# dvnam1605/MAACO-path-planing

Hardware: NVIDIA B200
Metric: path evals/sec (MAACO ant tours, MPA/PSO/GA fitness) at 1/2/4/8 B200 vs CPU (higher is better)
Workload: dtype f64

## Files before the change

maaco_path_planing_b200/csrc/mpp_maaco.cu:

```cuda
#include <type_traits>
#include <cmath>
#include <cstdlib>
#include <thread>
#include <vector>

#include "mpp_common.cuh"

static inline double hdist(int r0, int c0, int r1, int c1) {
    long long dr = r0 - r1, dc = c0 - c1;
    return std::sqrt((double)(dr * dr + dc * dc));
}

extern "C" double mpp_maaco_q0(int K, int k, double q0_initial) {
    double k0 = 0.7 * (double)K, q0;
    if ((double)k < k0) {
        if (std::fabs((double)K - k0) < 1e-6) q0 = q0_initial;
        else q0 = ((double)(K - k) / (double)K) * q0_initial;
    } else {
        double q0_at_k0 = (((double)K - k0) / (double)K) * q0_initial;
        q0 = q0_at_k0 +
             (((double)k - k0) / ((double)K - k0 + 1e-9)) * (q0_initial * (1 - ((double)K - k0) / (double)K) / 2.0);
    }
    q0 = q0 > 0.01 ? q0 : 0.01;
    return q0 < 0.99 ? q0 : 0.99;
}

static void host_tables(int R, int C, int start, int target, const mpp_maaco_params *p, double *tau0, double *E01,
                        double *dt) {
    const int sr = start / C, sc = start % C, tr = target / C, tc = target % C;
    double dsT = hdist(sr, sc, tr, tc);
    if (dsT < 1e-9) dsT = 1e-9;
    auto work = [&](int r_lo, int r_hi) {
        for (int r = r_lo; r < r_hi; ++r)
            for (int c = 0; c < C; ++c) {
                const size_t i = (size_t)r * C + c;
                const double diT = hdist(r, c, tr, tc);
                const double dsi = hdist(sr, sc, r, c);
                dt[i] = diT;
                {
                    const double den = dsi + diT;
                    double factor;
                    if (den < 1e-9) factor = (dsi < 1e-6 || diT < 1e-6) ? 1.0 : 0.1;
                    else factor = dsT / den;
                    const double v = factor * p->C0_initial_pheromone;
                    tau0[i] = v < 1e-9 ? 1e-9 : v;
                }
                double h;
                if (dsT < 1e-9) h = p->wh_min;
                else h = p->wh_max - (p->wh_max - p->wh_min) * std::exp(-p->k_h_adaptive * diT / dsT);
                const double g = 1.0 - h;
                const double base = g * dsi + h * diT;
                double d0 = base + p->a_turn_coef * 0.0, d1 = base + p->a_turn_coef * 1.0;
                d0 = d0 > 1e-9 ? d0 : 1e-9;
                d1 = d1 > 1e-9 ? d1 : 1e-9;
                E01[2 * i] = std::pow(1.0 / d0, p->beta);
                E01[2 * i + 1] = std::pow(1.0 / d1, p->beta);
            }
    };
    unsigned nt = std::thread::hardware_concurrency();
    if (nt > 16) nt = 16;
    if (nt < 2 || (size_t)R * C < 65536) {
        work(0, R);
    } else {
        std::vector<std::thread> th;
        int per = (R + (int)nt - 1) / (int)nt;
        for (unsigned t = 0; t < nt; ++t) {
            int lo = (int)t * per, hi = lo + per > R ? R : lo + per;
            if (lo < hi) th.emplace_back(work, lo, hi);
        }
        for (auto &t : th) t.join();
    }
}

__global__ void mpp_maaco_tau0_kernel(const double *__restrict__ tau0_free, const uint32_t *__restrict__ occ, int occ_words,
                                      int pitch, int R, int C, double *__restrict__ tau, long long tau_stride) {
    const int i = blockIdx.x * blockDim.x + threadIdx.x;
    if (i >= R * C) return;
    occ += (size_t)blockIdx.y * occ_words;
    const int r = i / C, pb = i % C + 1;
    const bool obst = (occ[(r + 1) * pitch + (pb >> 5)] >> (pb & 31)) & 1u;
    tau[(size_t)blockIdx.y * tau_stride + i] = obst ? 1e-9 : tau0_free[i];
}

extern "C" int mpp_maaco_tables(const mpp_map_batch *maps, const mpp_maaco_params *p, double *tau0_dev, long long tau_stride,
                                double *E01_dev, double *dist_t_dev, void *stream) {
    MPP_REQUIRE(maps && p && tau0_dev && E01_dev, "mpp_maaco_tables: null argument");
    const int R = maps->rows, C = maps->cols;
    const size_t n = (size_t)R * C;
    MPP_REQUIRE(tau_stride >= (long long)n, "mpp_maaco_tables: tau_stride < rows*cols");
    const MppMapMeta &M0 = maps->meta_host[0];
    MPP_REQUIRE(M0.start >= 0 && M0.target >= 0, "mpp_maaco_tables: map has no start/target");
    for (int k = 1; k < maps->n_maps; ++k)
        MPP_REQUIRE(maps->meta_host[k].start == M0.start && maps->meta_host[k].target == M0.target,
                    "mpp_maaco_tables: the maps of a batch must share start and target (map %d differs); group them", k);
    std::vector<double> buf(4 * n);
    double *tau0 = buf.data(), *E01 = tau0 + n, *dt = E01 + 2 * n;
    host_tables(R, C, M0.start, M0.target, p, tau0, E01, dt);
    cudaStream_t s = (cudaStream_t)stream;
    MPP_CUDA(cudaSetDevice(maps->device));
    double *tau0_free = nullptr;
    MPP_CUDA(cudaMalloc(&tau0_free, n * 8));
    MPP_CUDA(cudaMemcpyAsync(tau0_free, tau0, n * 8, cudaMemcpyHostToDevice, s));
    MPP_CUDA(cudaMemcpyAsync(E01_dev, E01, 2 * n * 8, cudaMemcpyHostToDevice, s));
    if (dist_t_dev) MPP_CUDA(cudaMemcpyAsync(dist_t_dev, dt, n * 8, cudaMemcpyHostToDevice, s));
    mpp_maaco_tau0_kernel<<<dim3(((int)n + 255) / 256, maps->n_maps), 256, 0, s>>>(
        tau0_free, maps->occ_dev, maps->occ_words, maps->pitch_words, R, C, tau0_dev, tau_stride);
    MPP_CUDA(cudaGetLastError());
    MPP_CUDA(cudaStreamSynchronize(s));
    MPP_CUDA(cudaFree(tau0_free));
    return MPP_OK;
}

struct RankLayout { size_t margin, fast_words, bundle_words, nb8_words, total_words; };
static RankLayout rank_layout(int R, int C) {
    RankLayout L;
    L.margin = (size_t)(C + 2) * 9;
    L.fast_words = ((size_t)9 * R * C + 2 * L.margin + 1) & ~(size_t)1;
    L.bundle_words = (L.fast_words + (size_t)18 * R * C + 3) & ~(size_t)3;
    L.nb8_words = L.bundle_words + (size_t)4 * R * C;
    L.total_words = L.nb8_words + (size_t)2 * R * C;
    return L;
}
static inline int tiles_r(int R) { return (R + 31) >> 5; }
static inline int tiles_c(int C) { return (C + 31) >> 5; }

extern "C" long long mpp_maaco_rank_words(int rows, int cols) { return (long long)rank_layout(rows, cols).total_words; }
extern "C" long long mpp_maaco_slab_words(int tile_rows, int cols, int n_ants) {
    return (long long)tile_rows * tiles_c(cols) * (long long)n_ants * 32;
}
extern "C" long long mpp_maaco_touched_words(int tile_rows, int cols, int n_ants) {
    return 2ll * tile_rows * tiles_c(cols) * ((n_ants + 31) / 32);
}

#define MPP_MAX_PEERS 16
struct TourArgs {
    const MppMapMeta *meta;
    const uint32_t *rank;
    size_t rank_stride, rank_margin, rank_fast_words, rank_bundle_words, rank_nb8_words;
    int R, C;
    const double *tau, *E01;
    size_t tau_stride, E01_stride;
    uint32_t it;
    double q0, alpha;
    int n_ants, ant_offset;
    const uint64_t *seeds;
    uint32_t *slabs, *touched;
    size_t slab_stride, touched_stride;
    uint8_t *moves;
    int max_cells;
    mpp_ant_result *result;
    size_t result_stride;
    unsigned long long *steps;
    const int32_t *latch;
};
struct TourPeers {
    uint32_t *peer_slabs[MPP_MAX_PEERS];
    uint32_t *peer_touched[MPP_MAX_PEERS];
    mpp_ant_result *peer_result[MPP_MAX_PEERS];
    int n_peers, rows_per_rank;
    int n_total;
};

#define MPP_SQRT2 1.4142135623730951
#ifndef MPP_TOUR1_THREADS
#define MPP_TOUR1_THREADS 128
#endif

__device__ __noinline__ double pow_slow(double x, double y) { return pow(x, y); }

__device__ __noinline__ int tour_select_slow(uint32_t cand, int cr, int cc, int C, bool have_prev, int prev_m,
                                             const double *__restrict__ tau, const double *__restrict__ E01,
                                             double alpha, double q0, double u0, double u1) {
    int mv[8], n = 0;
    double attr[8];
#pragma unroll
    for (int m = 0; m < 8; ++m) {
        if (!((cand >> m) & 1u)) continue;
        const int dr = (int)((0xA940u >> (2 * m)) & 3u) - 1, dc = (int)((0x9224u >> (2 * m)) & 3u) - 1;
        const int j = (cr + dr) * C + (cc + dc);
        const bool turn = have_prev && (m != prev_m);
        const double tv = tau[j];
        const double ta = (alpha == 1.0) ? tv : pow_slow(tv, alpha);
        attr[n] = ta * E01[2 * (size_t)j + (turn ? 1 : 0)];
        mv[n] = m;
        ++n;
    }
    int k;
    if (u0 <= q0) {
        double mx = -1.0;
        int best[8], nb = 0;
        for (int i = 0; i < n; ++i) {
            if (attr[i] > mx) { mx = attr[i]; nb = 0; best[nb++] = i; }
            else if (fabs(attr[i] - mx) < 1e-9) best[nb++] = i;
        }
        int q = (int)(u1 * (double)nb);
        q = q < nb ? q : nb - 1;
        k = best[q];
    } else {
        double S = 0.0;
        for (int i = 0; i < n; ++i) S += attr[i];
        bool uniform = S < 1e-9;
        double pr[8];
        double ps = 0.0;
        if (!uniform) {
            for (int i = 0; i < n; ++i) { pr[i] = attr[i] / S; ps += pr[i]; }
            if (fabs(ps - 1.0) > 1e-6) {
                const double ps0 = ps;
                ps = 0.0;
                for (int i = 0; i < n; ++i) { pr[i] = pr[i] / ps0; ps += pr[i]; }
            }
            if (!(fabs(ps - 1.0) <= 1.4901161193847656e-08)) uniform = true;
        }
        if (uniform) {
            k = (int)(u1 * (double)n);
        } else {
            double cdf[8], acc = 0.0;
            for (int i = 0; i < n; ++i) { acc += pr[i]; cdf[i] = acc; }
            k = 0;
            for (int i = 0; i < n; ++i)
                if (cdf[i] / acc <= u1) ++k;
        }
        k = k < n ? k : n - 1;
    }
    return mv[k];
}

struct TourSlabs {
    uint32_t *slabs, *touched;
    size_t n_ants;
    int NW, TR, TC;
    const TourPeers *peers;
    int rows_per_rank, ant_offset, NW_total;
    size_t n_total, peer_touched_off;
};
__device__ __forceinline__ uint32_t tour_tile_load(const TourSlabs &V, int a, int trow, int tcx, int lane) {
    if (trow < 0 || trow >= V.TR || tcx < 0 || tcx >= V.TC) return 0u;
    const int tile = trow * V.TC + tcx;
    uint32_t tw = 0u;
    if (lane == 0) tw = __ldcg(V.touched + (size_t)tile * V.NW + (a >> 5));
    tw = __shfl_sync(0xffffffffu, tw, 0);
    if (!((tw >> (a & 31)) & 1u)) return 0u;
    return __ldcg(V.slabs + ((size_t)tile * V.n_ants + a) * 32 + lane);
}
__device__ __forceinline__ void tour_tile_store(const TourSlabs &V, int a, int trow, int tcx, int lane, uint32_t v) {
    if (trow < 0 || trow >= V.TR || tcx < 0 || tcx >= V.TC) return;
    if (!__any_sync(0xffffffffu, v != 0u)) return;
    const int tile = trow * V.TC + tcx;
    V.slabs[((size_t)tile * V.n_ants + a) * 32 + lane] = v;
    if (lane == 0) atomicOr(V.touched + (size_t)tile * V.NW + (a >> 5), 1u << (a & 31));
    if (V.peers) {
        const int g = trow / V.rows_per_rank, tl = (trow - g * V.rows_per_rank) * V.TC + tcx;
        const size_t ga = (size_t)V.ant_offset + a;
        V.peers->peer_slabs[g][((size_t)tl * V.n_total + ga) * 32 + lane] = v;
        if (lane == 0) atomicOr(V.peers->peer_touched[g] + V.peer_touched_off + (size_t)tl * V.NW_total + (ga >> 5), 1u << (ga & 31));
    }
}

__device__ __forceinline__ uint32_t ldg32_pinned(const uint32_t *p) {
    uint32_t v;
    asm volatile("ld.volatile.global.u32 %0, [%1];" : "=r"(v) : "l"(p) : "memory");
    return v;
}
__device__ __forceinline__ uint2 lds_u2(uint32_t addr) {
    uint2 v;
    asm volatile("ld.shared.v2.u32 {%0, %1}, [%2];" : "=r"(v.x), "=r"(v.y) : "r"(addr));
    return v;
}
__device__ __forceinline__ uint32_t lds_u8(uint32_t addr) {
    uint32_t v;
    asm volatile("ld.shared.u8 %0, [%1];" : "=r"(v) : "r"(addr));
    return v;
}
__device__ __forceinline__ uint32_t lds_u32(uint32_t addr) {
// ... 366 lines not shown
                            pool = cand & ~((1u << best) - 1u);
                        }
                        const int n = __popc(pool);
                        const int k = (pack >> (3 * n - 3)) & 7u;
                        m = (int)lds_u8(sbase_k + T1_KTH_OFF + pool * 8u + (uint32_t)k);
                    }
                    const uint4 mvv = lds_u4(sbase_k + T1_MOVE_OFF + 16u * (uint32_t)m);
                    dcur = (int)mvv.x; dpr = (int)mvv.y; dcc = (int)mvv.z; dphi = (int)mvv.w;
                    dl = lds_f64(sbase_k + T1_DLEN_OFF + 8u * (uint32_t)m);
                    if (fast_ok) {
                        const uint32_t by = (((m & 4) ? nb.y : nb.x) >> (8 * (m & 3))) & 0xFFu;
                        const uint32_t fl = lds_u32(sbase_k + T1_FLD_OFF + 4u * (by >> 4));
                        const uint32_t A3n = (by >> 1) & 7u;
                        const uint32_t Gn = A3n ? ((fl >> (3u * (A3n - 1u))) & 7u) : 0u;
                        fw2 = (by & 1u) | (A3n << 1) | (fl << 4) | (Gn << 25);
                    }
                }
            }
            if (active) {
                cur += dcur;
                if (fast_ok) bq = ldg128_pinned(bundle + cur);
                gap -= dphi;
                gap = gap > 0 ? gap : 0;
                prow_s += (uint32_t)dpr;
                lrow += dpr >> 3;
                lcol += dcc;
                asm volatile("red.shared.or.b32 [%0], %1;" ::"r"(prow_s + 4u * ((uint32_t)lcol >> 5)), "r"(1u << (lcol & 31)) : "memory");
                if (n_path <= k_max_cells) *mvp = (uint8_t)m;
                ++mvp;
                len += dl;
                if (m != prev_m) ++turns;
                prev_m = m;
                ++n_path;
                if (cur == k_target || n_path >= k_max_path) active = false;
#ifdef MPP_TOUR_STATS
                st_c1 = clock64();
#endif
            }
        }
    }
    for (int src = 0; src < apw && a0 + src < A.n_ants; ++src) {
        const int s_wr = __shfl_sync(0xffffffffu, wr, src), s_wc = __shfl_sync(0xffffffffu, wc, src);
        const uint2 o0 = win_w[src * 64 + lane], o1 = win_w[src * 64 + lane + 32];
        tour_tile_store(V, a0 + src, s_wr, s_wc, lane, o0.x);
        tour_tile_store(V, a0 + src, s_wr, s_wc + 1, lane, o0.y);
        tour_tile_store(V, a0 + src, s_wr + 1, s_wc, lane, o1.x);
        tour_tile_store(V, a0 + src, s_wr + 1, s_wc + 1, lane, o1.y);
    }
    if (lane < apw && a < A.n_ants) {
        const bool ok = !failed && cur == target;
        mpp_ant_result res;
        res.length = ok ? len : __longlong_as_double(0x7ff0000000000000ll);
        res.n_cells = ok ? n_path : 0;
        res.turns = ok ? (turns > 0 ? turns : 0) : -1;
        A.result[(size_t)map * A.result_stride + A.ant_offset + a] = res;
        if constexpr (P2P)
            for (int g = 0; g < PA.n_peers; ++g) PA.peer_result[g][A.ant_offset + a] = res;
        if (A.steps) atomicAdd(A.steps, (unsigned long long)(n_path - 1));
#ifdef MPP_TOUR_STATS
        int *st = (int *)(A.moves + ((size_t)map * A.n_ants + a + 1) * A.max_cells - 32);
        st[0] = st_t1; st[1] = st_t2; st[2] = st_t3; st[3] = st_slides; st[4] = (int)(st_c1 - st_c0); st[5] = n_path - 1;
        st[6] = ok ? 1 : 0;
#endif
    }
}

static int colony_check(const mpp_map_batch *maps, const mpp_colony *c, const char *who) {
    MPP_REQUIRE(maps && c, "%s: null argument", who);
    MPP_REQUIRE(c->tau && c->E01 && c->rank && c->slabs && c->touched && c->moves && c->result && c->deposit && c->okbits &&
                    c->state && c->best_cells && c->seeds, "%s: null colony buffer", who);
    MPP_REQUIRE(c->max_cells > 0 && c->tau_stride >= (long long)maps->rows * maps->cols, "%s: bad max_cells / tau_stride", who);
    for (int k = 0; k < maps->n_maps; ++k)
        MPP_REQUIRE(maps->meta_host[k].start >= 0 && maps->meta_host[k].target >= 0, "%s: map %d has no start/target", who, k);
    return MPP_OK;
}

static int tours_launch(const mpp_map_batch *maps, const mpp_colony *c, int iteration, double q0, double alpha,
                        int n_ants, int ant_offset, int n_ants_total, int ants_per_warp,
                        uint32_t *const *peer_slabs, uint32_t *const *peer_touched, mpp_ant_result *const *peer_result,
                        int n_peers, int rows_per_rank, void *stream) {
    int rc = colony_check(maps, c, "mpp_maaco_tours");
    if (rc) return rc;
    MPP_REQUIRE(n_ants > 0 && ant_offset >= 0 && ant_offset + n_ants <= n_ants_total, "mpp_maaco_tours: bad ant range");
    MPP_CUDA(cudaSetDevice(maps->device));
    const RankLayout L = rank_layout(maps->rows, maps->cols);
    const int TR = tiles_r(maps->rows);
    TourArgs A;
    A.meta = maps->meta_dev;
    A.rank = c->rank; A.rank_stride = L.total_words; A.rank_margin = L.margin; A.rank_fast_words = L.fast_words;
    A.rank_bundle_words = L.bundle_words; A.rank_nb8_words = L.nb8_words;
    A.R = maps->rows; A.C = maps->cols;
    A.tau = c->tau; A.tau_stride = (size_t)c->tau_stride; A.E01 = c->E01; A.E01_stride = (size_t)c->E01_stride;
    A.it = (uint32_t)iteration; A.q0 = q0; A.alpha = alpha;
    A.n_ants = n_ants; A.ant_offset = ant_offset;
    A.seeds = c->seeds;
    const size_t tw = (size_t)mpp_maaco_touched_words(TR, maps->cols, n_ants) / 2;
    A.slabs = c->slabs; A.slab_stride = (size_t)mpp_maaco_slab_words(TR, maps->cols, n_ants);
    A.touched = c->touched + (size_t)(iteration & 1) * tw * maps->n_maps; A.touched_stride = tw;
    A.moves = c->moves; A.max_cells = c->max_cells;
    A.result = c->result; A.result_stride = (size_t)n_ants_total;
    A.steps = c->steps; A.latch = c->latch;
    TourPeers PA;
    for (int g = 0; g < MPP_MAX_PEERS; ++g) {
        PA.peer_slabs[g] = g < n_peers ? peer_slabs[g] : nullptr;
        PA.peer_touched[g] = g < n_peers ? peer_touched[g] : nullptr;
        PA.peer_result[g] = g < n_peers ? peer_result[g] : nullptr;
    }
    PA.n_peers = n_peers; PA.rows_per_rank = rows_per_rank; PA.n_total = n_ants_total;
    int apw = 16;
    const char *e = getenv("MPP_TOUR_APW");
    if (e) apw = atoi(e);
    else if (ants_per_warp) apw = ants_per_warp;
    else {
        const long long total = (long long)n_ants * maps->n_maps;
        while (apw > 2 && (total + apw - 1) / apw < 12ll * maps->sm_count) apw >>= 1;
    }
    MPP_REQUIRE(apw == 1 || apw == 2 || apw == 4 || apw == 8 || apw == 16 || apw == 32,
                "ants per warp (MPP_TOUR_APW / ants_per_warp) must be a power of two <= 32");
    const int warps = (n_ants + apw - 1) / apw, wpb = MPP_TOUR1_THREADS / 32;
    const size_t smem = T1_WIN_OFF + (size_t)wpb * apw * 512;
    {
        static size_t smem_set[64] = {0};
        const int dv = maps->device & 63;
        if (smem > smem_set[dv]) {
            MPP_CUDA(cudaFuncSetAttribute(mpp_maaco_tour1_kernel<false>, cudaFuncAttributeMaxDynamicSharedMemorySize, (int)smem));
            MPP_CUDA(cudaFuncSetAttribute(mpp_maaco_tour1_kernel<true>, cudaFuncAttributeMaxDynamicSharedMemorySize, (int)smem));
            smem_set[dv] = smem;
        }
    }
    const dim3 grid((warps + wpb - 1) / wpb, maps->n_maps);
    if (n_peers > 0) mpp_maaco_tour1_kernel<true><<<grid, MPP_TOUR1_THREADS, smem, (cudaStream_t)stream>>>(A, apw, PA);
    else mpp_maaco_tour1_kernel<false><<<grid, MPP_TOUR1_THREADS, smem, (cudaStream_t)stream>>>(A, apw, TourNoPeers());
    MPP_CUDA(cudaGetLastError());
    return MPP_OK;
}

extern "C" int mpp_maaco_tours(const mpp_map_batch *maps, const mpp_colony *c, int iteration, double q0, double alpha,
                               int n_ants, int ant_offset, int n_ants_total, int ants_per_warp, void *stream) {
    return tours_launch(maps, c, iteration, q0, alpha, n_ants, ant_offset, n_ants_total, ants_per_warp, nullptr, nullptr,
                        nullptr, 0, 1, stream);
}

extern "C" int mpp_maaco_tours_p2p(const mpp_map_batch *maps, const mpp_colony *c, int iteration, double q0, double alpha,
                                   int n_ants, int ant_offset, int n_ants_total, int ants_per_warp,
                                   uint32_t *const *slabs_peers, uint32_t *const *touched_peers,
                                   mpp_ant_result *const *result_peers, int n_peers, int tile_rows_per_rank, void *stream) {
    MPP_REQUIRE(maps && maps->n_maps == 1, "mpp_maaco_tours_p2p: a sharded colony is one map");
    MPP_REQUIRE(slabs_peers && touched_peers && result_peers && n_peers > 0 && n_peers <= MPP_MAX_PEERS && tile_rows_per_rank > 0 &&
                    (long long)n_peers * tile_rows_per_rank >= tiles_r(maps->rows), "mpp_maaco_tours_p2p: bad peer arguments");
    return tours_launch(maps, c, iteration, q0, alpha, n_ants, ant_offset, n_ants_total, ants_per_warp, slabs_peers,
                        touched_peers, result_peers, n_peers, tile_rows_per_rank, stream);
}

__global__ void __launch_bounds__(128) mpp_maaco_rank_kernel(const uint8_t *__restrict__ svalid_all,
                                                             const double *__restrict__ tau_all, size_t tau_stride,
                                                             const double *__restrict__ E01_all, size_t E01_stride,
                                                             double alpha, int R, int C,
                                                             const MppMapMeta *__restrict__ meta, uint32_t *__restrict__ rank_all,
                                                             size_t rank_stride, size_t rank_margin, size_t rank_fast_words,
                                                             size_t rank_bundle_words, size_t rank_nb8_words,
                                                             const int32_t *__restrict__ latch) {
    const int cell = blockIdx.x * 128 + threadIdx.x;
    if (cell >= R * C) return;
    if (latch && *latch) return;
    const int map = blockIdx.y;
    const uint8_t *svalid = svalid_all + (size_t)map * R * C;
    const double *tau = tau_all + (size_t)map * tau_stride;
    const double *E01 = E01_all + (size_t)map * E01_stride;
    uint32_t *rank_fast = rank_all + (size_t)map * rank_stride + rank_margin;
    uint2 *rank_slow = (uint2 *)(rank_all + (size_t)map * rank_stride + rank_fast_words);
    uint32_t *bundle = rank_all + (size_t)map * rank_stride + rank_bundle_words;
    uint8_t *nb8 = (uint8_t *)(rank_all + (size_t)map * rank_stride + rank_nb8_words);
    const uint32_t P1 = meta[map].s1.P1;
    const uint32_t sv = svalid[cell];
    double a0[8], a1[8];
#pragma unroll
    for (int m = 0; m < 8; ++m) {
        a0[m] = a1[m] = -1.0;
        if ((sv >> m) & 1u) {
            const int j = cell + ((int)((0xA940u >> (2 * m)) & 3u) - 1) * C + ((int)((0x9224u >> (2 * m)) & 3u) - 1);
            const double tv = tau[j];
            const double ta = (alpha == 1.0) ? tv : pow_slow(tv, alpha);
            const double2 e = *(const double2 *)(E01 + 2 * (size_t)j);
            a0[m] = ta * e.x;
            a1[m] = ta * e.y;
        }
    }
    const bool p1_three = __popc(P1) == 3;
    const int s0 = __ffs(P1) - 1, s1 = __ffs(P1 & (P1 - 1)) - 1, s2 = 31 - __clz(P1);
    for (int ctx = 0; ctx < 9; ++ctx) {
        double a[8];
#pragma unroll
        for (int m = 0; m < 8; ++m) a[m] = (ctx > 0 && m != ctx - 1) ? a1[m] : a0[m];
        double cmx = 0.0;
#pragma unroll
        for (int m = 0; m < 8; ++m) cmx = fmax(cmx, a[m]);
        uint32_t word = 0xFFFFFFu, perm = 0u, fast = 7u, order = 0u;
        if (cmx < 1e-10) {
            word = 0u;
#pragma unroll
            for (int m = 0; m < 8; ++m) {
                int pos = 0;
#pragma unroll
                for (int q = 0; q < 8; ++q) pos += (a[q] > a[m]) || (a[q] == a[m] && q < m);
                word |= (uint32_t)pos << (3 * m);
                perm |= (uint32_t)m << (4 * pos);
            }
            fast = 0u;
            if (p1_three) {
                const uint32_t p0 = (word >> (3 * s0)) & 7u, p1 = (word >> (3 * s1)) & 7u, p2 = (word >> (3 * s2)) & 7u;
                order = (p0 < p1 ? 1u : 0u) | (p0 < p2 ? 2u : 0u) | (p1 < p2 ? 4u : 0u);
#pragma unroll
                for (uint32_t c = 1; c < 8; ++c) {
                    uint32_t bp = 8u, bi = 0u;
                    if ((c & 1u) && p0 < bp) { bp = p0; bi = 0u; }
                    if ((c & 2u) && p1 < bp) { bp = p1; bi = 1u; }
                    if ((c & 4u) && p2 < bp) { bp = p2; bi = 2u; }
                    fast |= (c & ~((1u << bi) - 1u)) << (3u * c);
                }
            }
        }
        const size_t t = (size_t)cell * 9 + ctx;
        rank_fast[t] = fast | (sv << 24);
        rank_slow[t] = make_uint2(perm, word | (sv << 24));
        if (p1_three && ctx > 0) {
            const int mv = ctx - 1;
            const int pr = cell / C - ((int)((0xA940u >> (2 * mv)) & 3u) - 1), pc = cell % C - ((int)((0x9224u >> (2 * mv)) & 3u) - 1);
            if (pr >= 0 && pr < R && pc >= 0 && pc < C) {
                const uint32_t A3 = ((sv >> s0) & 1u) | (((sv >> s1) & 1u) << 1) | (((sv >> s2) & 1u) << 2);
                nb8[((size_t)pr * C + pc) * 8 + mv] = (uint8_t)((fast & 7u ? 1u : 0u) | (A3 << 1) | (order << 4));
                const int k = (ctx == s0 + 1) ? 0 : ((ctx == s1 + 1) ? 1 : ((ctx == s2 + 1) ? 2 : -1));
                if (k >= 0) bundle[((size_t)pr * C + pc) * 4 + k] = tour_word2(fast | (sv << 24), s0, s1, s2);
            }
        }
    }
}

extern "C" int mpp_maaco_rank(const mpp_map_batch *maps, const mpp_colony *c, double alpha, void *stream) {
    int rc = colony_check(maps, c, "mpp_maaco_rank");
    if (rc) return rc;
    MPP_CUDA(cudaSetDevice(maps->device));
    const int total = maps->rows * maps->cols;
    const RankLayout L = rank_layout(maps->rows, maps->cols);
    mpp_maaco_rank_kernel<<<dim3((total + 127) / 128, maps->n_maps), 128, 0, (cudaStream_t)stream>>>(
        maps->svalid_dev, c->tau, (size_t)c->tau_stride, c->E01, (size_t)c->E01_stride, alpha, maps->rows, maps->cols,
        maps->meta_dev, c->rank, L.total_words, L.margin, L.fast_words, L.bundle_words, L.nb8_words, c->latch);
    MPP_CUDA(cudaGetLastError());
    return MPP_OK;
}

#define MPP_BEST_THREADS 1024
__device__ __forceinline__ bool lt_len_idx(double la, int ia, double lb, int ib) {
    return la < lb || (la == lb && ia < ib);
}
__device__ __forceinline__ int move_delta(uint32_t m, int C) {
    return ((int)((0xA940u >> (2 * m)) & 3u) - 1) * C + ((int)((0x9224u >> (2 * m)) & 3u) - 1);
}

__global__ void __launch_bounds__(MPP_BEST_THREADS)
mpp_maaco_best_kernel(const mpp_ant_result *__restrict__ res_all, const uint8_t *__restrict__ moves_all, int max_cells,
                      int moves_ant_offset, int moves_n_ants, int n, double Q, int iteration, int C,
                      const MppMapMeta *__restrict__ meta, mpp_maaco_state *state_all, int32_t *best_cells_all,
                      double *deposit_all, uint32_t *okbits_all, double *log_all, int log_rows,
                      const int32_t *__restrict__ latch) {
    __shared__ double s_len[32];
    __shared__ int s_idx[32];
    __shared__ int s_t[32];
    __shared__ double b_len;
    __shared__ int b_r, b_ant, b_turns, b_copy, s_base;
    if (latch && *latch) return;
    const int map = blockIdx.x;
    const mpp_ant_result *res = res_all + (size_t)map * n;
    double *deposit = deposit_all + (size_t)map * n;
    uint32_t *okbits = okbits_all + (size_t)map * ((n + 31) >> 5);
    mpp_maaco_state *state = state_all + map;
    const int tid = threadIdx.x, lane = tid & 31, wid = tid >> 5;
    const double INF = __longlong_as_double(0x7ff0000000000000ll);
    double ml = INF;
    int mi = 0x7fffffff;
    for (int i0 = 0; i0 < n; i0 += MPP_BEST_THREADS) {
        const int i = i0 + tid;
        bool dep = false;
        if (i < n) {
            const mpp_ant_result ri = res[i];
            const double l = ri.length;
            if (lt_len_idx(l, i, ml, mi)) { ml = l; mi = i; }
            dep = (l != INF && ri.n_cells > 0 && l > 1e-6);
            deposit[i] = dep ? Q / l : 0.0;
        }
        const uint32_t ok = __ballot_sync(0xffffffffu, dep);
        if (lane == 0 && i < n) okbits[i >> 5] = ok;
    }
#pragma unroll
    for (int o = 16; o; o >>= 1) {
        const double ol = __shfl_xor_sync(0xffffffffu, ml, o);
        const int oi = __shfl_xor_sync(0xffffffffu, mi, o);
        if (lt_len_idx(ol, oi, ml, mi)) { ml = ol; mi = oi; }
    }
    if (lane == 0) { s_len[wid] = ml; s_idx[wid] = mi; }
    __syncthreads();
    if (wid == 0) {
        ml = s_len[lane]; mi = s_idx[lane];
#pragma unroll
        for (int o = 16; o; o >>= 1) {
            const double ol = __shfl_xor_sync(0xffffffffu, ml, o);
            const int oi = __shfl_xor_sync(0xffffffffu, mi, o);
            if (lt_len_idx(ol, oi, ml, mi)) { ml = ol; mi = oi; }
        }
        if (lane == 0) { b_len = ml; b_r = mi; }
    }
    __syncthreads();
    const double L = b_len;
    const int r = b_r;
    int bt = 0x7fffffff, bi = 0x7fffffff;
    if (L != INF) {
        for (int i = tid; i < n; i += MPP_BEST_THREADS) {
            if (i < r) continue;
            const mpp_ant_result ri = res[i];
            const double l = ri.length;
            if (i == r || fabs(l - L) < 1e-9) {
                const int t = ri.turns;
                if (t >= 0 && (t < bt || (t == bt && i < bi))) { bt = t; bi = i; }
            }
        }
    }
#pragma unroll
    for (int o = 16; o; o >>= 1) {
        const int ot = __shfl_xor_sync(0xffffffffu, bt, o), oi = __shfl_xor_sync(0xffffffffu, bi, o);
        if (ot < bt || (ot == bt && oi < bi)) { bt = ot; bi = oi; }
    }
    if (lane == 0) { s_t[wid] = bt; s_idx[wid] = bi; }
    __syncthreads();
    if (wid == 0) {
        bt = s_t[lane]; bi = s_idx[lane];
#pragma unroll
        for (int o = 16; o; o >>= 1) {
            const int ot = __shfl_xor_sync(0xffffffffu, bt, o), oi = __shfl_xor_sync(0xffffffffu, bi, o);
            if (ot < bt || (ot == bt && oi < bi)) { bt = ot; bi = oi; }
        }
        if (lane == 0) {
            const bool any = (L != INF);
            b_ant = any ? bi : -1;
            b_turns = any ? bt : -1;
            mpp_maaco_state st = *state;
            int copy = 0;
            if (any) {
                if (L < st.best_len) {
                    st.best_len = L; st.best_turns = bt; copy = 1;
                } else if (fabs(L - st.best_len) < 1e-9) {
                    if (bt < st.best_turns) { st.best_turns = bt; copy = 1; }
                }
            }
            if (copy) { st.best_n_cells = res[bi].n_cells; st.best_iter = iteration; st.best_ant = bi; }
            st.iter_best_len = L; st.iter_best_turns = b_turns; st.iter_best_ant = b_ant;
            *state = st;
            b_copy = copy;
            if (log_all && iteration >= 1 && iteration <= log_rows) {
                double *lg = log_all + ((size_t)map * log_rows + (size_t)(iteration - 1)) * 4;
                lg[0] = L; lg[1] = (double)b_turns; lg[2] = st.best_len; lg[3] = (double)st.best_turns;
            }
        }
    }
    __syncthreads();
    if (b_copy && b_ant >= moves_ant_offset && b_ant < moves_ant_offset + moves_n_ants) {
        const int a = b_ant - moves_ant_offset;
        int nm = res[b_ant].n_cells - 1;
        if (nm > max_cells) nm = max_cells;
        const uint8_t *mv = moves_all + ((size_t)map * moves_n_ants + a) * max_cells;
        int32_t *out = best_cells_all + (size_t)map * (max_cells + 1);
        if (tid == 0) { out[0] = meta[map].start; s_base = meta[map].start; }
        __syncthreads();
        for (int k0 = 0; k0 < nm; k0 += MPP_BEST_THREADS) {
            const int k = k0 + tid;
            int x = (k < nm) ? move_delta(mv[k], C) : 0;
#pragma unroll
            for (int o = 1; o < 32; o <<= 1) { const int y = __shfl_up_sync(0xffffffffu, x, o); if (lane >= o) x += y; }
            if (lane == 31) s_idx[wid] = x;
            __syncthreads();
            if (wid == 0) {
                int w = s_idx[lane];
#pragma unroll
                for (int o = 1; o < 32; o <<= 1) { const int y = __shfl_up_sync(0xffffffffu, w, o); if (lane >= o) w += y; }
                s_idx[lane] = w;
            }
            __syncthreads();
            const int cell = s_base + (wid ? s_idx[wid - 1] : 0) + x;
            if (k < nm) out[k + 1] = cell;
            __syncthreads();
            if (tid == MPP_BEST_THREADS - 1) s_base = cell;
            __syncthreads();
        }
    }
}

extern "C" int mpp_maaco_best(const mpp_map_batch *maps, const mpp_colony *c, int moves_ant_offset, int moves_n_ants,
                              int n_ants_total, double Q, int iteration, void *stream) {
    int rc = colony_check(maps, c, "mpp_maaco_best");
// ... 481 lines not shown
```

Baseline: 5.982 million.

## Tile MAACO rank kernel in shared memory with incremental ranking and coalesced stores

Rewrites the rank kernel to process 32x8 cell tiles. Each block stages tau^alpha*E01 products in shared memory with a halo, so each neighbour's product is computed once per tile rather than once per adjacent cell. The per-context 8x8 rank comparison is replaced by precomputed rank words with an incremental fix-up for the changed move. Outputs are staged in shared memory so fast/slow rank words and nb8/bundle entries go out as coalesced row writes instead of scattered byte stores. This costs a halo recompute for border cells, extra shared memory and more register pressure, and the logic is intricate enough to risk ranking mismatches.

```diff
diff --git a/maaco_path_planing_b200/csrc/mpp_maaco.cu b/maaco_path_planing_b200/csrc/mpp_maaco.cu
--- a/maaco_path_planing_b200/csrc/mpp_maaco.cu
+++ b/maaco_path_planing_b200/csrc/mpp_maaco.cu
@@ -118,7 +118,7 @@
     L.fast_words = ((size_t)9 * R * C + 2 * L.margin + 1) & ~(size_t)1;
     L.bundle_words = (L.fast_words + (size_t)18 * R * C + 3) & ~(size_t)3;
     L.nb8_words = L.bundle_words + (size_t)4 * R * C;
-    L.total_words = L.nb8_words + (size_t)2 * R * C;
+    L.total_words = (L.nb8_words + (size_t)2 * R * C + 3) & ~(size_t)3;
     return L;
 }
 static inline int tiles_r(int R) { return (R + 31) >> 5; }
@@ -791,7 +791,26 @@
                         touched_peers, result_peers, n_peers, tile_rows_per_rank, stream);
 }
 
-__global__ void __launch_bounds__(128) mpp_maaco_rank_kernel(const uint8_t *__restrict__ svalid_all,
+#define RANK_TW 32
+#define RANK_TH 8
+#define RANK_EW (RANK_TW + 2)
+#define RANK_EH (RANK_TH + 2)
+#define RANK_AW (RANK_TW + 4)
+#define RANK_AH (RANK_TH + 4)
+#ifndef MPP_RANK_MINB
+#define MPP_RANK_MINB 4
+#endif
+
+__device__ __forceinline__ int rank_beats(double aq, double am, bool q_lower) { return q_lower ? (aq >= am) : (aq > am); }
+
+__device__ __forceinline__ uint32_t rank_word2_of_byte(uint32_t by, const uint32_t *fields) {
+    const uint32_t A3 = (by >> 1) & 7u;
+    if (by & 1u) return 1u | (A3 << 1);
+    const uint32_t f = fields[by >> 4];
+    return (A3 << 1) | (f << 4) | ((A3 ? (f >> (3u * (A3 - 1u))) & 7u : 0u) << 25);
+}
+
+__global__ void __launch_bounds__(RANK_TW * RANK_TH, MPP_RANK_MINB) mpp_maaco_rank_kernel(const uint8_t *__restrict__ svalid_all,
                                                              const double *__restrict__ tau_all, size_t tau_stride,
                                                              const double *__restrict__ E01_all, size_t E01_stride,
                                                              double alpha, int R, int C,
@@ -799,89 +818,188 @@
                                                              size_t rank_stride, size_t rank_margin, size_t rank_fast_words,
                                                              size_t rank_bundle_words, size_t rank_nb8_words,
                                                              const int32_t *__restrict__ latch) {
-    const int cell = blockIdx.x * 128 + threadIdx.x;
-    if (cell >= R * C) return;
+    __shared__ double2 s_a[RANK_AH][RANK_AW];
+    __shared__ uint2 s_nb[RANK_EH][RANK_EW];
+    __shared__ uint32_t s_fast[RANK_TH][RANK_TW * 9];
+    __shared__ uint2 s_slow[RANK_TH][RANK_TW * 9];
+    __shared__ uint32_t s_fields[8];
     if (latch && *latch) return;
-    const int map = blockIdx.y;
+    const int map = blockIdx.y, tid = threadIdx.x, lane = tid & 31, wid = tid >> 5;
+    const int TCn = (C + RANK_TW - 1) / RANK_TW;
+    const int r0 = (blockIdx.x / TCn) * RANK_TH, c0 = (blockIdx.x % TCn) * RANK_TW;
     const uint8_t *svalid = svalid_all + (size_t)map * R * C;
     const double *tau = tau_all + (size_t)map * tau_stride;
     const double *E01 = E01_all + (size_t)map * E01_stride;
     uint32_t *rank_fast = rank_all + (size_t)map * rank_stride + rank_margin;
     uint2 *rank_slow = (uint2 *)(rank_all + (size_t)map * rank_stride + rank_fast_words);
-    uint32_t *bundle = rank_all + (size_t)map * rank_stride + rank_bundle_words;
-    uint8_t *nb8 = (uint8_t *)(rank_all + (size_t)map * rank_stride + rank_nb8_words);
+    uint4 *bundle = (uint4 *)(rank_all + (size_t)map * rank_stride + rank_bundle_words);
+    uint2 *nb8 = (uint2 *)(rank_all + (size_t)map * rank_stride + rank_nb8_words);
     const uint32_t P1 = meta[map].s1.P1;
-    const uint32_t sv = svalid[cell];
-    double a0[8], a1[8];
-#pragma unroll
-    for (int m = 0; m < 8; ++m) {
-        a0[m] = a1[m] = -1.0;
-        if ((sv >> m) & 1u) {
-            const int j = cell + ((int)((0xA940u >> (2 * m)) & 3u) - 1) * C + ((int)((0x9224u >> (2 * m)) & 3u) - 1);
+    const bool p1_three = __popc(P1) == 3;
+    const int s0 = __ffs(P1) - 1, s1 = __ffs(P1 & (P1 - 1)) - 1, s2 = 31 - __clz(P1);
+    if (tid < 8) s_fields[tid] = tour_fields(tid);
+    for (int i = tid; i < RANK_AH * RANK_AW; i += RANK_TW * RANK_TH) {
+        const int r = r0 - 2 + i / RANK_AW, c = c0 - 2 + i % RANK_AW;
+        double2 v = make_double2(-1.0, -1.0);
+        if (r >= 0 && r < R && c >= 0 && c < C) {
+            const size_t j = (size_t)r * C + c;
             const double tv = tau[j];
             const double ta = (alpha == 1.0) ? tv : pow_slow(tv, alpha);
-            const double2 e = *(const double2 *)(E01 + 2 * (size_t)j);
-            a0[m] = ta * e.x;
-            a1[m] = ta * e.y;
-        }
-    }
-    const bool p1_three = __popc(P1) == 3;
-    const int s0 = __ffs(P1) - 1, s1 = __ffs(P1 & (P1 - 1)) - 1, s2 = 31 - __clz(P1);
-    for (int ctx = 0; ctx < 9; ++ctx) {
-        double a[8];
-#pragma unroll
-        for (int m = 0; m < 8; ++m) a[m] = (ctx > 0 && m != ctx - 1) ? a1[m] : a0[m];
-        double cmx = 0.0;
-#pragma unroll
-        for (int m = 0; m < 8; ++m) cmx = fmax(cmx, a[m]);
-        uint32_t word = 0xFFFFFFu, perm = 0u, fast = 7u, order = 0u;
-        if (cmx < 1e-10) {
-            word = 0u;
-#pragma unroll
-            for (int m = 0; m < 8; ++m) {
-                int pos = 0;
-#pragma unroll
-                for (int q = 0; q < 8; ++q) pos += (a[q] > a[m]) || (a[q] == a[m] && q < m);
-                word |= (uint32_t)pos << (3 * m);
-                perm |= (uint32_t)m << (4 * pos);
-            }
-            fast = 0u;
-            if (p1_three) {
-                const uint32_t p0 = (word >> (3 * s0)) & 7u, p1 = (word >> (3 * s1)) & 7u, p2 = (word >> (3 * s2)) & 7u;
-                order = (p0 < p1 ? 1u : 0u) | (p0 < p2 ? 2u : 0u) | (p1 < p2 ? 4u : 0u);
-#pragma unroll
-                for (uint32_t c = 1; c < 8; ++c) {
-                    uint32_t bp = 8u, bi = 0u;
-                    if ((c & 1u) && p0 < bp) { bp = p0; bi = 0u; }
-                    if ((c & 2u) && p1 < bp) { bp = p1; bi = 1u; }
-                    if ((c & 4u) && p2 < bp) { bp = p2; bi = 2u; }
-                    fast |= (c & ~((1u << bi) - 1u)) << (3u * c);
-                }
-            }
-        }
-        const size_t t = (size_t)cell * 9 + ctx;
-        rank_fast[t] = fast | (sv << 24);
-        rank_slow[t] = make_uint2(perm, word | (sv << 24));
-        if (p1_three && ctx > 0) {
-            const int mv = ctx - 1;
-            const int pr = cell / C - ((int)((0xA940u >> (2 * mv)) & 3u) - 1), pc = cell % C - ((int)((0x9224u >> (2 * mv)) & 3u) - 1);
-            if (pr >= 0 && pr < R && pc >= 0 && pc < C) {
-                const uint32_t A3 = ((sv >> s0) & 1u) | (((sv >> s1) & 1u) << 1) | (((sv >> s2) & 1u) << 2);
-                nb8[((size_t)pr * C + pc) * 8 + mv] = (uint8_t)((fast & 7u ? 1u : 0u) | (A3 << 1) | (order << 4));
-                const int k = (ctx == s0 + 1) ? 0 : ((ctx == s1 + 1) ? 1 : ((ctx == s2 + 1) ? 2 : -1));
-                if (k >= 0) bundle[((size_t)pr * C + pc) * 4 + k] = tour_word2(fast | (sv << 24), s0, s1, s2);
-            }
-        }
-    }
+            const double2 e = *(const double2 *)(E01 + 2 * j);
+            v = make_double2(ta * e.x, ta * e.y);
+        }
+        s_a[i / RANK_AW][i % RANK_AW] = v;
+    }
+    __syncthreads();
+    for (int i = tid; i < RANK_EH * RANK_EW; i += RANK_TW * RANK_TH) {
+        int er, ec;
+        if (i < RANK_TW * RANK_TH) { er = i / RANK_TW + 1; ec = i % RANK_TW + 1; }
+        else {
+            const int h = i - RANK_TW * RANK_TH;
+            if (h < RANK_EW) { er = 0; ec = h; }
+            else if (h < 2 * RANK_EW) { er = RANK_EH - 1; ec = h - RANK_EW; }
+            else if (h < 2 * RANK_EW + RANK_TH) { er = h - 2 * RANK_EW + 1; ec = 0; }
+            else { er = h - 2 * RANK_EW - RANK_TH + 1; ec = RANK_EW - 1; }
+        }
+        const int r = r0 - 1 + er, c = c0 - 1 + ec;
+        const bool inner = er >= 1 && er <= RANK_TH && ec >= 1 && ec <= RANK_TW;
+        if (r < 0 || r >= R || c < 0 || c >= C) { s_nb[er][ec] = make_uint2(0u, 0u); continue; }
+        const uint32_t sv = svalid[(size_t)r * C + c];
+        double a0[8], a1[8];
+#pragma unroll
+        for (int m = 0; m < 8; ++m) {
+            a0[m] = a1[m] = -1.0;
+            if ((sv >> m) & 1u) {
+                const int dr = (int)((0xA940u >> (2 * m)) & 3u) - 1, dc = (int)((0x9224u >> (2 * m)) & 3u) - 1;
+                const double2 v = s_a[er + 1 + dr][ec + 1 + dc];
+                a0[m] = v.x;
+                a1[m] = v.y;
+            }
+        }
+        uint32_t big0 = 0u, big1 = 0u;
+        const uint32_t A3 = ((sv >> s0) & 1u) | (((sv >> s1) & 1u) << 1) | (((sv >> s2) & 1u) << 2);
+        if (!inner) {
+            if (!p1_three) { s_nb[er][ec] = make_uint2(0u, 0u); continue; }
+            double sum = 0.0;
+#pragma unroll
+            for (int q = 0; q < 8; ++q) {
+                big0 |= (a0[q] >= 1e-10 ? 1u : 0u) << q;
+                big1 |= (a1[q] >= 1e-10 ? 1u : 0u) << q;
+                sum += a0[q] + a1[q];
+            }
+            if (sum == sum) {
+                double m0[3], m1[3];
+#pragma unroll
+                for (int k = 0; k < 3; ++k) {
+                    const int mv = k == 0 ? s0 : (k == 1 ? s1 : s2);
+                    const int dr = (int)((0xA940u >> (2 * mv)) & 3u) - 1, dc = (int)((0x9224u >> (2 * mv)) & 3u) - 1;
+                    const double2 v = ((sv >> mv) & 1u) ? s_a[er + 1 + dr][ec + 1 + dc] : make_double2(-1.0, -1.0);
+                    m0[k] = v.x;
+                    m1[k] = v.y;
+                }
+                uint2 nbw = make_uint2(0u, 0u);
+#pragma unroll
+                for (int p = 0; p < 8; ++p) {
+                    const bool applies = ((big1 & ~(1u << p)) | (big0 & (1u << p))) == 0u;
+                    const double w0 = p == s0 ? m0[0] : m1[0], w1 = p == s1 ? m0[1] : m1[1], w2 = p == s2 ? m0[2] : m1[2];
+                    const uint32_t order = (w0 >= w1 ? 1u : 0u) | (w0 >= w2 ? 2u : 0u) | (w1 >= w2 ? 4u : 0u);
+                    const uint32_t by = (applies ? order << 4 : 1u) | (A3 << 1);
+                    if (p < 4) nbw.x |= by << (8 * p); else nbw.y |= by << (8 * (p - 4));
+                }
+                s_nb[er][ec] = nbw;
+                continue;
+            }
+            big0 = big1 = 0u;
+        }
+        uint32_t R0[8], R1[8], word0 = 0u, word1 = 0u;
+#pragma unroll
+        for (int q = 0; q < 8; ++q) {
+            big0 |= (a0[q] >= 1e-10 ? 1u : 0u) << q;
+            big1 |= (a1[q] >= 1e-10 ? 1u : 0u) << q;
+            R0[q] = R1[q] = 0u;
+#pragma unroll
+            for (int m = 0; m < 8; ++m)
+                if (m != q) {
+                    R0[q] |= (uint32_t)rank_beats(a0[q], a0[m], q < m) << (3 * m);
+                    R1[q] |= (uint32_t)rank_beats(a1[q], a1[m], q < m) << (3 * m);
+                }
+            word0 += R0[q];
+            word1 += R1[q];
+        }
+        uint2 nbw = make_uint2(0u, 0u);
+#pragma unroll
+        for (int ctx = 0; ctx < 9; ++ctx) {
+            const int p = ctx - 1;
+            const bool applies = ctx == 0 ? big0 == 0u : (((big1 & ~(1u << p)) | (big0 & (1u << p))) == 0u);
+            uint32_t word = 0xFFFFFFu, perm = 0u, fast = 7u, order = 0u;
+            if (applies) {
+                if (ctx == 0) {
+                    word = word0;
+                } else {
+                    uint32_t X = 0u, pp = 0u;
+#pragma unroll
+                    for (int m = 0; m < 8; ++m)
+                        if (m != p) {
+                            X |= (uint32_t)rank_beats(a0[p], a1[m], p < m) << (3 * m);
+                            pp += (uint32_t)rank_beats(a1[m], a0[p], m < p);
+                        }
+                    word = word1 - R1[p] + X - (((word1 >> (3 * p)) & 7u) << (3 * p)) + (pp << (3 * p));
+                }
+                if (inner) {
+#pragma unroll
+                    for (int m = 0; m < 8; ++m) perm |= (uint32_t)m << (4 * ((word >> (3 * m)) & 7u));
+                }
+                fast = 0u;
+                if (p1_three) {
+                    const uint32_t q0 = (word >> (3 * s0)) & 7u, q1 = (word >> (3 * s1)) & 7u, q2 = (word >> (3 * s2)) & 7u;
+                    order = (q0 < q1 ? 1u : 0u) | (q0 < q2 ? 2u : 0u) | (q1 < q2 ? 4u : 0u);
+                    fast = s_fields[order] << 3;
+                }
+            }
+            if (inner) {
+                s_fast[er - 1][(ec - 1) * 9 + ctx] = fast | (sv << 24);
+                s_slow[er - 1][(ec - 1) * 9 + ctx] = make_uint2(perm, word | (sv << 24));
+            }
+            if (ctx > 0) {
+                const uint32_t by = (fast & 7u ? 1u : 0u) | (A3 << 1) | (order << 4);
+                if (p < 4) nbw.x |= by << (8 * p); else nbw.y |= by << (8 * (p - 4));
+            }
+        }
+        s_nb[er][ec] = nbw;
+    }
+    __syncthreads();
+    const int r = r0 + wid;
+    if (r >= R) return;
+    const int nrow = (C - c0 < RANK_TW ? C - c0 : RANK_TW) * 9;
+    const size_t e0 = ((size_t)r * C + c0) * 9;
+    for (int i = lane; i < nrow; i += 32) {
+        rank_fast[e0 + i] = s_fast[wid][i];
+        rank_slow[e0 + i] = s_slow[wid][i];
+    }
+    const int c = c0 + lane;
+    if (!p1_three || c >= C) return;
+    uint2 row = make_uint2(0u, 0u);
+#pragma unroll
+    for (int m = 0; m < 8; ++m) {
+        const int dr = (int)((0xA940u >> (2 * m)) & 3u) - 1, dc = (int)((0x9224u >> (2 * m)) & 3u) - 1;
+        const uint2 w = s_nb[wid + 1 + dr][lane + 1 + dc];
+        const uint32_t by = ((m < 4 ? w.x : w.y) >> (8 * (m & 3))) & 0xFFu;
+        if (m < 4) row.x |= by << (8 * m); else row.y |= by << (8 * (m - 4));
+    }
+    const size_t cell = (size_t)r * C + c;
+    nb8[cell] = row;
+    auto byte_of = [&](int m) { return ((m < 4 ? row.x : row.y) >> (8 * (m & 3))) & 0xFFu; };
+    bundle[cell] = make_uint4(rank_word2_of_byte(byte_of(s0), s_fields), rank_word2_of_byte(byte_of(s1), s_fields),
+                              rank_word2_of_byte(byte_of(s2), s_fields), 0u);
 }
 
 extern "C" int mpp_maaco_rank(const mpp_map_batch *maps, const mpp_colony *c, double alpha, void *stream) {
     int rc = colony_check(maps, c, "mpp_maaco_rank");
     if (rc) return rc;
     MPP_CUDA(cudaSetDevice(maps->device));
-    const int total = maps->rows * maps->cols;
     const RankLayout L = rank_layout(maps->rows, maps->cols);
-    mpp_maaco_rank_kernel<<<dim3((total + 127) / 128, maps->n_maps), 128, 0, (cudaStream_t)stream>>>(
+    const int tiles = ((maps->rows + RANK_TH - 1) / RANK_TH) * ((maps->cols + RANK_TW - 1) / RANK_TW);
+    mpp_maaco_rank_kernel<<<dim3(tiles, maps->n_maps), RANK_TW * RANK_TH, 0, (cudaStream_t)stream>>>(
         maps->svalid_dev, c->tau, (size_t)c->tau_stride, c->E01, (size_t)c->E01_stride, alpha, maps->rows, maps->cols,
         maps->meta_dev, c->rank, L.total_words, L.margin, L.fast_words, L.bundle_words, L.nb8_words, c->latch);
     MPP_CUDA(cudaGetLastError());
```

Result: faster. 6.113 million, median of 6 (+2.2%).
